# Kudo510/ImageSequenceRegistrationfor6DPoseEstimationLabeling

Hardware: AMD Instinct MI355X
Metric: registered images/sec (T-LESS obj 1-like, synthetic) + final Chamfer error (higher is better)
Workload: dtype bf16

## Files before the change

imagesequenceregistrationfor6dposeestimationlabeling_amd/csrc/nn_batched.hip:

```cpp
#include "isr_common.hpp"

#include <cstddef>
#include <cstdlib>

namespace {

#ifndef ISR_NN_PACKED_BATCH
#define ISR_NN_PACKED_BATCH 1
#endif
constexpr int kThreads = 256;
constexpr int kTile = 256;
constexpr int kGroup = 8;
constexpr int kNV = 18;

__device__ __forceinline__ void xform64(const double* __restrict__ T, float x, float y, float z,
                                        double& ox, double& oy, double& oz) {
  if (T == nullptr) {
    ox = x; oy = y; oz = z;
    return;
  }
  const double dx = x, dy = y, dz = z;
  ox = fma(T[2], dz, fma(T[1], dy, fma(T[0], dx, T[3])));
  oy = fma(T[6], dz, fma(T[5], dy, fma(T[4], dx, T[7])));
  oz = fma(T[10], dz, fma(T[9], dy, fma(T[8], dx, T[11])));
}

constexpr int kUnresolved = -2;

template <int RQ>
__device__ __forceinline__ int query_of(int r) {
  return (int)blockIdx.x * RQ * kThreads + ((int)threadIdx.x >> 6) * (RQ * 64) + r * 64 + ((int)threadIdx.x & 63);
}

__global__ __launch_bounds__(256) void tile_box_kernel(const float* __restrict__ tgt, int Nt, float* __restrict__ box) {
  __shared__ float red[6][4];
  const int j = blockIdx.x * 256 + threadIdx.x;
  float v[6] = {3.0e38f, 3.0e38f, 3.0e38f, -3.0e38f, -3.0e38f, -3.0e38f};
  if (j < Nt) {
#pragma unroll
    for (int a = 0; a < 3; ++a) v[a] = v[3 + a] = tgt[3 * (size_t)j + a];
  }
#pragma unroll
  for (int a = 0; a < 3; ++a) {
#pragma unroll
    for (int o = 32; o >= 1; o >>= 1) {
      v[a] = fminf(v[a], __shfl_xor(v[a], o, 64));
      v[3 + a] = fmaxf(v[3 + a], __shfl_xor(v[3 + a], o, 64));
    }
  }
  if ((threadIdx.x & 63) == 0) {
#pragma unroll
    for (int a = 0; a < 6; ++a) red[a][threadIdx.x >> 6] = v[a];
  }
  __syncthreads();
  if (threadIdx.x < 6) {
    const int a = threadIdx.x;
    const float r0 = red[a][0], r1 = red[a][1], r2 = red[a][2], r3 = red[a][3];
    box[6 * (size_t)blockIdx.x + a] = a < 3 ? fminf(fminf(r0, r1), fminf(r2, r3)) : fmaxf(fmaxf(r0, r1), fmaxf(r2, r3));
  }
}

constexpr int kIcpItemDoubles = 20;
constexpr int kIcpStateInts = 8;
template <int RQ, bool FILTER, bool EXACT = false, bool CULL = false, bool ITEMS = false>
__global__ __launch_bounds__(kThreads) void nn_search_kernel(
    const float* __restrict__ qry, int Nq, const float* __restrict__ tgt, int Nt,
    const double* __restrict__ Tq, const double* __restrict__ Tt, int split_len, int nsplit,
    float* __restrict__ part_d2, int32_t* __restrict__ part_idx, const int32_t* __restrict__ skip,
    const int32_t* __restrict__ unresolved, unsigned long long* __restrict__ packed = nullptr,
    const int32_t* __restrict__ warm = nullptr, int32_t* __restrict__ amb = nullptr,
    const float* __restrict__ t2_bound = nullptr, const float* __restrict__ tile_box = nullptr, float cull_r2 = 0.f,
    size_t qry_item_stride = 0) {
  __shared__ __attribute__((aligned(16))) float lds[2][FILTER ? 4 : 3][kTile];
  __shared__ float tile_t2[2][kThreads / 64];
  if (ITEMS) {
    if (skip[(size_t)blockIdx.z * kIcpStateInts]) return;
    qry += (size_t)blockIdx.z * qry_item_stride;
  } else if (skip && *skip) {
    return;
  }
  if (unresolved && *unresolved == 0) return;

  const int tid = threadIdx.x;
  const int b = blockIdx.z;
  const int split = blockIdx.y;
  if (unresolved) {
    int mine = 0;
#pragma unroll
    for (int r = 0; r < RQ; ++r) {
      const int qi = query_of<RQ>(r);
      if (qi < Nq) mine |= part_idx[((size_t)b * nsplit + split) * Nq + qi] == kUnresolved;
// ... 326 lines not shown
      counted = (radius < 0.0) || (s2 <= radius * radius);
      if (counted) {
        v[0] = d; v[1] = s2; v[2] = 1.0;
        if (WANT_COV) {
          const double q[3] = {q0, q1, q2}, t[3] = {t0, t1, t2};
#pragma unroll
          for (int r = 0; r < 3; ++r) {
            v[3 + r] = q[r];
            v[6 + r] = t[r];
#pragma unroll
            for (int c = 0; c < 3; ++c) v[9 + 3 * r + c] = q[r] * t[c];
          }
        }
      }
    }
    if (nn_idx) nn_idx[(size_t)b * Nq + qi] = counted ? bi : -1;
    if (nn_d) nn_d[(size_t)b * Nq + qi] = d;
  }

  constexpr int nv = WANT_COV ? kNV : 3;
  const int wave = tid >> 6, lane = tid & 63;
#pragma unroll
  for (int k = 0; k < nv; ++k) {
    const double s = wave_sum(v[k]);
    if (lane == 0) red[wave][k] = s;
  }
  __syncthreads();
  if (tid < kNV) {
    double s = 0.0;
    if (tid < nv) s = ((red[0][tid] + red[1][tid]) + red[2][tid]) + red[3][tid];
    part_sums[((size_t)b * gridDim.x + blockIdx.x) * kNV + tid] = s;
  }
}

__global__ void nn_reduce_kernel(const double* __restrict__ part_sums, int nblk, int B,
                                 double* __restrict__ sum_d, double* __restrict__ sum_d2,
                                 int32_t* __restrict__ n_in, double* __restrict__ cov) {
  const int b = blockIdx.x * blockDim.y + threadIdx.y;
  const int k = threadIdx.x;
  if (b >= B || k >= kNV) return;
  double s = 0.0;
  for (int i = 0; i < nblk; ++i) s += part_sums[((size_t)b * nblk + i) * kNV + k];
  if (k == 0 && sum_d) sum_d[b] = s;
  if (k == 1 && sum_d2) sum_d2[b] = s;
  if (k == 2 && n_in) n_in[b] = (int32_t)s;
  if (k >= 3 && cov) cov[(size_t)b * 16 + (k - 3)] = s;
  if (k == 2 && cov) cov[(size_t)b * 16 + 15] = s;
}


__global__ __launch_bounds__(kThreads) void add_metric_kernel(const float* __restrict__ verts, int V,
                                                              const double* __restrict__ Ta,
                                                              const double* __restrict__ Tb,
                                                              double* __restrict__ out) {
  __shared__ double red[kThreads / 64];
  const int b = blockIdx.x;
  const double* ta = Ta ? Ta + 12 * (size_t)b : nullptr;
  const double* tb = Tb ? Tb + 12 * (size_t)b : nullptr;
  double s = 0.0;
  for (int i = threadIdx.x; i < V; i += kThreads) {
    const float x = verts[3 * (size_t)i], y = verts[3 * (size_t)i + 1], z = verts[3 * (size_t)i + 2];
    double a0, a1, a2, b0, b1, b2;
    xform64(ta, x, y, z, a0, a1, a2);
    xform64(tb, x, y, z, b0, b1, b2);
    const double ex = a0 - b0, ey = a1 - b1, ez = a2 - b2;
    s += sqrt(fma(ez, ez, fma(ey, ey, ex * ex)));
  }
  s = wave_sum(s);
  if ((threadIdx.x & 63) == 0) red[threadIdx.x >> 6] = s;
  __syncthreads();
  if (threadIdx.x == 0) out[b] = (((red[0] + red[1]) + red[2]) + red[3]) / (double)V;
}


struct IcpState {
  double prev_fit, prev_rmse;
  int32_t iter, done;
  int32_t ticket, pad;
};
static_assert(sizeof(IcpState) == kIcpStateInts * sizeof(int32_t) && offsetof(IcpState, done) == 5 * sizeof(int32_t),
              "nn_search_kernel<.., ITEMS> steps from one item's done flag to the next by kIcpStateInts");

__device__ void jacobi4_largest(double A[4][4], double q[4]) {
  double V[4][4] = {{1, 0, 0, 0}, {0, 1, 0, 0}, {0, 0, 1, 0}, {0, 0, 0, 1}};
  for (int sweep = 0; sweep < 16; ++sweep) {
    double off = 0.0, dia = 0.0;
#pragma unroll
    for (int p = 0; p < 4; ++p) {
      dia += A[p][p] * A[p][p];
#pragma unroll
      for (int r = p + 1; r < 4; ++r) off += A[p][r] * A[p][r];
    }
    if (off <= 1e-34 * dia) break;
#pragma unroll
    for (int p = 0; p < 3; ++p)
#pragma unroll
      for (int r = p + 1; r < 4; ++r) {
        if (A[p][r] != 0.0) {
          const double theta = (A[r][r] - A[p][p]) / (2.0 * A[p][r]);
          const double t = (theta >= 0 ? 1.0 : -1.0) / (fabs(theta) + sqrt(theta * theta + 1.0));
          const double c = 1.0 / sqrt(t * t + 1.0), sn = t * c;
#pragma unroll
          for (int k = 0; k < 4; ++k) {
            const double akp = A[k][p], akr = A[k][r];
            A[k][p] = c * akp - sn * akr;
            A[k][r] = sn * akp + c * akr;
          }
#pragma unroll
          for (int k = 0; k < 4; ++k) {
            const double apk = A[p][k], ark = A[r][k];
            A[p][k] = c * apk - sn * ark;
            A[r][k] = sn * apk + c * ark;
          }
#pragma unroll
          for (int k = 0; k < 4; ++k) {
            const double vkp = V[k][p], vkr = V[k][r];
            V[k][p] = c * vkp - sn * vkr;
            V[k][r] = sn * vkp + c * vkr;
          }
        }
      }
  }
  double lam = A[0][0];
#pragma unroll
  for (int k = 0; k < 4; ++k) q[k] = V[k][0];
#pragma unroll
  for (int j = 1; j < 4; ++j) {
    if (A[j][j] > lam) {
      lam = A[j][j];
#pragma unroll
      for (int k = 0; k < 4; ++k) q[k] = V[k][j];
    }
  }
}

constexpr int kIcpLanes = 16;

__device__ void icp_reduce_and_update(const double* __restrict__ part_sums, int nblk, int Ns, int max_iter,
                                      double rel_fitness, double rel_rmse, double* __restrict__ T,
                                      IcpState* __restrict__ st, double* __restrict__ result) {
  __shared__ double part[kNV][kIcpLanes];
  __shared__ double v[kNV];
  for (int idx = threadIdx.x; idx < kNV * kIcpLanes; idx += blockDim.x) {
    const int k = idx / kIcpLanes, l = idx % kIcpLanes;
    double s = 0.0;
    for (int i = l; i < nblk; i += kIcpLanes) s += part_sums[(size_t)i * kNV + k];
    part[k][l] = s;
  }
  __syncthreads();
  if (threadIdx.x < kNV) {
    double s = 0.0;
    for (int l = 0; l < kIcpLanes; ++l) s += part[threadIdx.x][l];
    v[threadIdx.x] = s;
  }
  __syncthreads();
  if (threadIdx.x != 0) return;
  const double n = v[2];
  const double fit = n / (double)Ns;
  const double rmse = n > 0 ? sqrt(v[1] / n) : 0.0;
  const int it = st->iter;
  result[0] = fit; result[1] = rmse; result[2] = (double)it; result[3] = n;
  const bool conv = it > 0 && fabs(st->prev_fit - fit) < rel_fitness && fabs(st->prev_rmse - rmse) < rel_rmse;
  if (conv || it >= max_iter || n < 3) { st->done = 1; return; }
  st->prev_fit = fit; st->prev_rmse = rmse; st->iter = it + 1;
  double mq[3], mt[3], S[3][3];
  for (int a = 0; a < 3; ++a) { mq[a] = v[3 + a] / n; mt[a] = v[6 + a] / n; }
  for (int a = 0; a < 3; ++a)
    for (int b = 0; b < 3; ++b) S[a][b] = v[9 + 3 * a + b] - n * mq[a] * mt[b];
  double N4[4][4] = {
      {S[0][0] + S[1][1] + S[2][2], S[1][2] - S[2][1], S[2][0] - S[0][2], S[0][1] - S[1][0]},
      {S[1][2] - S[2][1], S[0][0] - S[1][1] - S[2][2], S[0][1] + S[1][0], S[2][0] + S[0][2]},
      {S[2][0] - S[0][2], S[0][1] + S[1][0], -S[0][0] + S[1][1] - S[2][2], S[1][2] + S[2][1]},
      {S[0][1] - S[1][0], S[2][0] + S[0][2], S[1][2] + S[2][1], -S[0][0] - S[1][1] + S[2][2]}};
  double q[4];
  jacobi4_largest(N4, q);
  const double nq = 1.0 / sqrt(q[0] * q[0] + q[1] * q[1] + q[2] * q[2] + q[3] * q[3]);
  const double w = q[0] * nq, x = q[1] * nq, y = q[2] * nq, z = q[3] * nq;
  const double R[3][3] = {{1 - 2 * (y * y + z * z), 2 * (x * y - z * w), 2 * (x * z + y * w)},
                          {2 * (x * y + z * w), 1 - 2 * (x * x + z * z), 2 * (y * z - x * w)},
                          {2 * (x * z - y * w), 2 * (y * z + x * w), 1 - 2 * (x * x + y * y)}};
  double U[3][4];
  for (int a = 0; a < 3; ++a) {
    for (int b = 0; b < 3; ++b) U[a][b] = R[a][b];
    U[a][3] = mt[a] - (R[a][0] * mq[0] + R[a][1] * mq[1] + R[a][2] * mq[2]);
  }
  double Tn[12];
  for (int a = 0; a < 3; ++a)
    for (int b = 0; b < 4; ++b)
      Tn[4 * a + b] = U[a][0] * T[b] + U[a][1] * T[4 + b] + U[a][2] * T[8 + b] + (b == 3 ? U[a][3] : 0.0);
  for (int k = 0; k < 12; ++k) T[k] = Tn[k];
}

__global__ __launch_bounds__(kThreads) void icp_finalize_update_kernel(
    const float* __restrict__ src, int Ns, const float* __restrict__ tgt, int Nt, double radius,
    unsigned long long* __restrict__ packed, int32_t* __restrict__ prev_idx, int32_t* __restrict__ amb,
    double* __restrict__ part_sums, int max_iter,
    double rel_fitness, double rel_rmse, double* __restrict__ T, IcpState* __restrict__ st, double* __restrict__ result,
    size_t src_item_stride = 0, size_t out_item_stride = 0) {
  __shared__ double red[kThreads / 64][kNV];
  __shared__ int last;
  __shared__ int nflag, flist[kThreads];
  __shared__ double wd[4][kThreads / 64];
  __shared__ int wi[4][kThreads / 64];
  {
    const size_t b = blockIdx.y;
    src += b * src_item_stride;
    packed += b * Ns; prev_idx += b * Ns; amb += b * Ns;
    part_sums += b * gridDim.x * kNV;
    st += b;
    T += b * out_item_stride; result += b * out_item_stride;
  }
  if (st->done) return;
  const int tid = threadIdx.x;
  const int qi = blockIdx.x * kThreads + tid;
  if (tid == 0) nflag = 0;
  __syncthreads();
  if (qi < Ns && amb[qi]) {
    amb[qi] = 0;
    flist[atomicAdd(&nflag, 1)] = qi;
  }
  __syncthreads();
  const int nf = nflag;
  constexpr int kRes = 4;
  for (int f0 = 0; f0 < nf; f0 += kRes) {
    double qx[kRes], qy[kRes], qz[kRes], bd[kRes];
    int bi[kRes];
#pragma unroll
    for (int k = 0; k < kRes; ++k) {
      const int pq = flist[min(f0 + k, nf - 1)];
      xform64(T, src[3 * (size_t)pq], src[3 * (size_t)pq + 1], src[3 * (size_t)pq + 2], qx[k], qy[k], qz[k]);
      bd[k] = __builtin_inf();
      bi[k] = 0x7fffffff;
    }
#pragma unroll 4
    for (int j = tid; j < Nt; j += kThreads) {
      const double tx = tgt[3 * (size_t)j], ty = tgt[3 * (size_t)j + 1], tz = tgt[3 * (size_t)j + 2];
#pragma unroll
      for (int k = 0; k < kRes; ++k) {
        const double ex = qx[k] - tx, ey = qy[k] - ty, ez = qz[k] - tz;
        const double s2 = fma(ez, ez, fma(ey, ey, ex * ex));
        if (s2 < bd[k]) { bd[k] = s2; bi[k] = j; }
      }
    }
#pragma unroll
    for (int k = 0; k < kRes; ++k) {
#pragma unroll
      for (int off = 32; off > 0; off >>= 1) {
        const double od = __shfl_xor(bd[k], off, 64);
        const int oi = __shfl_xor(bi[k], off, 64);
        if (od < bd[k] || (od == bd[k] && oi < bi[k])) { bd[k] = od; bi[k] = oi; }
      }
      if ((tid & 63) == 0) { wd[k][tid >> 6] = bd[k]; wi[k][tid >> 6] = bi[k]; }
    }
    __syncthreads();
    if (tid < kRes && f0 + tid < nf) {
      double d = wd[tid][0];
      int i = wi[tid][0];
      for (int w = 1; w < kThreads / 64; ++w)
        if (wd[tid][w] < d || (wd[tid][w] == d && wi[tid][w] < i)) { d = wd[tid][w]; i = wi[tid][w]; }
      packed[flist[f0 + tid]] = ((unsigned long long)__float_as_uint((float)d) << 32) | (unsigned int)i;
    }
    __syncthreads();
  }
  double v[kNV];
#pragma unroll
  for (int k = 0; k < kNV; ++k) v[k] = 0.0;
  if (qi < Ns) {
    const unsigned long long pk = packed[qi];
    packed[qi] = ~0ull;
    prev_idx[qi] = pk != ~0ull ? (int)(unsigned int)pk : -1;
    if (pk != ~0ull) {
      const int bi = (int)(unsigned int)pk;
      double q0, q1, q2;
      xform64(T, src[3 * (size_t)qi], src[3 * (size_t)qi + 1], src[3 * (size_t)qi + 2], q0, q1, q2);
      const double t0 = tgt[3 * (size_t)bi], t1 = tgt[3 * (size_t)bi + 1], t2 = tgt[3 * (size_t)bi + 2];
      const double ex = q0 - t0, ey = q1 - t1, ez = q2 - t2;
      const double s2 = fma(ez, ez, fma(ey, ey, ex * ex));
      if (s2 <= radius * radius) {
        v[0] = sqrt(s2); v[1] = s2; v[2] = 1.0;
        const double q[3] = {q0, q1, q2}, t[3] = {t0, t1, t2};
#pragma unroll
        for (int r = 0; r < 3; ++r) {
          v[3 + r] = q[r];
          v[6 + r] = t[r];
#pragma unroll
          for (int c = 0; c < 3; ++c) v[9 + 3 * r + c] = q[r] * t[c];
        }
      }
    }
  }
  const int wave = tid >> 6, lane = tid & 63;
#pragma unroll
  for (int k = 0; k < kNV; ++k) {
    const double s = wave_sum(v[k]);
    if (lane == 0) red[wave][k] = s;
  }
  __syncthreads();
  if (tid < kNV) part_sums[(size_t)blockIdx.x * kNV + tid] = ((red[0][tid] + red[1][tid]) + red[2][tid]) + red[3][tid];
  __threadfence();
  __syncthreads();
  if (tid == 0) last = (atomicAdd(&st->ticket, 1) == (int)gridDim.x - 1);
  __syncthreads();
  if (!last) return;
  __threadfence();
  if (tid == 0) st->ticket = 0;
  icp_reduce_and_update(part_sums, gridDim.x, Ns, max_iter, rel_fitness, rel_rmse, T, st, result);
}

__global__ void icp_init_kernel(IcpState* st, double* T, unsigned long long* packed, int32_t* amb, int Ns,
                                size_t out_item_stride = 0) {
  const size_t b = blockIdx.y;
  const int i = blockIdx.x * blockDim.x + threadIdx.x;
  if (i < Ns) { packed[b * Ns + i] = ~0ull; amb[b * Ns + i] = 0; }
  if (i != 0) return;
  st += b; T += b * out_item_stride;
  st->prev_fit = 0; st->prev_rmse = 0; st->iter = 0; st->done = 0; st->ticket = 0;
  T[12] = 0; T[13] = 0; T[14] = 0; T[15] = 1;
}

__global__ __launch_bounds__(kThreads) void cloud_r2max_kernel(const float* __restrict__ tgt, int Nt, float* __restrict__ out) {
  __shared__ float red[kThreads / 64];
  float m = 0.f;
  for (int j = threadIdx.x; j < Nt; j += kThreads) {
    const float x = tgt[3 * (size_t)j], y = tgt[3 * (size_t)j + 1], z = tgt[3 * (size_t)j + 2];
    m = fmaxf(m, __builtin_fmaf(z, z, __builtin_fmaf(y, y, x * x)));
  }
#pragma unroll
  for (int o = 32; o >= 1; o >>= 1) m = fmaxf(m, __shfl_xor(m, o, 64));
  if ((threadIdx.x & 63) == 0) red[threadIdx.x >> 6] = m;
  __syncthreads();
  if (threadIdx.x == 0) *out = 1.0001f * fmaxf(fmaxf(red[0], red[1]), fmaxf(red[2], red[3]));
}

struct NNPlan {
  int rq;
  int qblocks;
  int nsplit;
  int split_len;
  int fblocks;
  int bchunk;
  bool grid;
  bool tile;
};

constexpr size_t kPartBudget = size_t(192) << 20;

NNPlan make_plan(int Nq, int Nt, int B, bool brute_only = false) {
  NNPlan p;
  p.rq = (Nq >= 4 * kThreads) ? 4 : 1;
  const int rq_knob = isr::tuning(ISR_TUNE_NN_PLAN_RQ);
  const long want_env = isr::tuning(ISR_TUNE_NN_PLAN_BLOCKS);
  if (rq_knob == 1 || rq_knob == 4) p.rq = rq_knob;
  p.qblocks = (Nq + p.rq * kThreads - 1) / (p.rq * kThreads);
#ifndef ISR_NN_WANT_BLOCKS
#define ISR_NN_WANT_BLOCKS 4096
#endif
  const long want = want_env > 0 ? want_env : ISR_NN_WANT_BLOCKS;
  long ns = (want + (long)p.qblocks * B - 1) / ((long)p.qblocks * B);
  const int max_split = (Nt + kTile - 1) / kTile;
  if (ns < 1) ns = 1;
  if (ns > max_split) ns = max_split;
  int tiles_per_split = (max_split + (int)ns - 1) / (int)ns;
  p.split_len = tiles_per_split * kTile;
  p.nsplit = (Nt + p.split_len - 1) / p.split_len;
  p.fblocks = (Nq + kThreads - 1) / kThreads;
  p.grid = false;
  p.tile = B >= 4 && Nq >= 1024 && Nt >= 4096 && (long)Nq * B >= (1L << 17);
  if (const int path = isr::tuning(ISR_TUNE_NN_PATH); path >= 0) { p.grid = path == 1; p.tile = path == 2; }
  if (brute_only) p.grid = p.tile = false;
  if (p.grid || p.tile) {
    p.nsplit = 1;
    p.split_len = max_split * kTile;
  }
  const size_t per_b = (size_t)p.nsplit * Nq * 8;
  long bc = (long)(kPartBudget / (per_b ? per_b : 1));
  if (bc < 1) bc = 1;
  if (bc > B) bc = B;
  if (bc > 65535) bc = 65535;
  p.bchunk = (int)bc;
  return p;
}

constexpr int kFilterMinTiles = 4;
void launch_search(const NNPlan& p, const dim3& grid, hipStream_t stream, const float* qry, int Nq, const float* tgt, int Nt,
                   const double* tq, const double* tt, float* part_d2, int32_t* part_idx, const int32_t* skip,
                   const int32_t* unresolved, unsigned long long* packed, const int32_t* warm, int32_t* amb = nullptr,
                   const float* t2_bound = nullptr, const float* tile_box = nullptr, float cull_r2 = 0.f,
                   bool items = false, size_t qry_item_stride = 0) {
  bool filter = warm != nullptr || p.split_len >= kFilterMinTiles * kTile;
  if (const int f = isr::tuning(ISR_TUNE_NN_FILTER); f >= 0 && !warm) filter = f == 1;
#define ISR_SEARCH(RQv, Fv)                                                                                              \
  nn_search_kernel<RQv, Fv><<<grid, kThreads, 0, stream>>>(qry, Nq, tgt, Nt, tq, tt, p.split_len, p.nsplit, part_d2, part_idx, \
                                                           skip, unresolved, packed, warm)
#define ISR_SEARCH_X(RQv, Fv)                                                                                            \
  nn_search_kernel<RQv, Fv, true, Fv><<<grid, kThreads, 0, stream>>>(qry, Nq, tgt, Nt, tq, tt, p.split_len, p.nsplit, part_d2, \
                                                                     part_idx, skip, unresolved, packed, warm, amb, t2_bound, tile_box, cull_r2)
#define ISR_SEARCH_ITEMS(RQv, Fv)                                                                                        \
  nn_search_kernel<RQv, Fv, true, Fv, true><<<grid, kThreads, 0, stream>>>(qry, Nq, tgt, Nt, tq, tt, p.split_len, p.nsplit,    \
                                                                           part_d2, part_idx, skip, unresolved, packed, warm, \
                                                                           amb, t2_bound, tile_box, cull_r2, qry_item_stride)
  if (items) {
    if (p.rq == 4) { if (filter) ISR_SEARCH_ITEMS(4, true); else ISR_SEARCH_ITEMS(4, false); }
    else { if (filter) ISR_SEARCH_ITEMS(1, true); else ISR_SEARCH_ITEMS(1, false); }
    return;
  }
  if (amb) {
    if (p.rq == 4) { if (filter) ISR_SEARCH_X(4, true); else ISR_SEARCH_X(4, false); }
    else { if (filter) ISR_SEARCH_X(1, true); else ISR_SEARCH_X(1, false); }
    return;
  }
  if (p.rq == 4) { if (filter) ISR_SEARCH(4, true); else ISR_SEARCH(4, false); }
  else { if (filter) ISR_SEARCH(1, true); else ISR_SEARCH(1, false); }
#undef ISR_SEARCH_ITEMS
#undef ISR_SEARCH_X
#undef ISR_SEARCH
}

}

extern "C" size_t isr_nn_batched_workspace_bytes(int Nq, int Nt, int B) {
  if (Nq <= 0 || Nt <= 0 || B <= 0) return 0;
  const NNPlan p = make_plan(Nq, Nt, B);
  size_t n = 0;
  n += isr::align_up((size_t)p.bchunk * p.nsplit * Nq * sizeof(float), 256);
  n += isr::align_up((size_t)p.bchunk * p.nsplit * Nq * sizeof(int32_t), 256);
  n += isr::align_up((size_t)B * p.fblocks * kNV * sizeof(double), 256);
  if (p.grid) n += grid_ws_bytes(Nt);
  if (p.tile) n += tile_ws_bytes(Nq, Nt);
  return n + 256;
}

extern "C" int isr_nn_batched(const float* qry, int Nq, const float* tgt, int Nt, const double* Tq,
// ... 19 lines not shown
  TileWs tw{};
  if (p.grid) {
    gw = take_grid(w, Nt);
    build_grid(gw, tgt, Nt, stream);
    ISR_CHECK_LAUNCH("grid build");
  }
  if (p.tile) {
    tw = take_tile(w, Nq, Nt);
    build_tile(tw, qry, Nq, tgt, Nt, stream);
    ISR_CHECK_LAUNCH("tile grid build");
  }
  const float stop_radius = (radius >= 0.0 && !nn_d) ? (float)(radius * (1.0 + 1e-6)) : -1.f;

  for (int b0 = 0; b0 < B; b0 += p.bchunk) {
    const int nb = (B - b0 < p.bchunk) ? (B - b0) : p.bchunk;
    const double* tq = Tq ? Tq + 12 * (size_t)b0 : nullptr;
    const double* tt = Tt ? Tt + 12 * (size_t)b0 : nullptr;
    const dim3 grid(p.qblocks, p.nsplit, nb);
    const int32_t* unres = nullptr;
    if (p.grid) {
      nn_grid_search_kernel<<<dim3(p.fblocks, nb), kThreads, 0, stream>>>(qry, Nq, gw.desc, gw.start, gw.sorted, tq, tt,
                                                                          stop_radius, part_d2, part_idx,
                                                                          gw.unresolved, nullptr);
      ISR_CHECK_LAUNCH("nn_grid_search_kernel");
      unres = gw.unresolved;
    }
    unsigned long long* packed = nullptr;
    if (!p.tile && !p.grid && p.nsplit > 1 && ISR_NN_PACKED_BATCH) {
      packed = reinterpret_cast<unsigned long long*>(part_d2);
      ISR_CHECK_HIP(hipMemsetAsync(packed, 0xFF, (size_t)nb * Nq * sizeof(unsigned long long), stream));
    }
    if (p.tile)
      launch_tile_search(tw, Nq, Nt, tq, tt, nb, stop_radius, part_d2, part_idx, nullptr, stream);
    else
      launch_search(p, grid, stream, qry, Nq, tgt, Nt, tq, tt, packed ? nullptr : part_d2, packed ? nullptr : part_idx, nullptr, unres,
                    packed, nullptr);
    ISR_CHECK_LAUNCH("nn_search_kernel");
    const dim3 fgrid(p.fblocks, nb);
    if (cov)
      nn_finalize_kernel<true><<<fgrid, kThreads, 0, stream>>>(qry, Nq, tgt, Tq, Tt, p.nsplit,
                                                               radius, part_d2, part_idx, b0,
                                                               nn_idx, nn_d, part_sums, nullptr, packed);
    else
      nn_finalize_kernel<false><<<fgrid, kThreads, 0, stream>>>(qry, Nq, tgt, Tq, Tt, p.nsplit,
                                                                radius, part_d2, part_idx, b0,
                                                                nn_idx, nn_d, part_sums, nullptr, packed);
    ISR_CHECK_LAUNCH("nn_finalize_kernel");
  }
  if (sum_d || sum_d2 || n_in || cov) {
    const dim3 rblock(32, 8);
    nn_reduce_kernel<<<(B + 7) / 8, rblock, 0, stream>>>(part_sums, p.fblocks, B, sum_d, sum_d2,
                                                         n_in, cov);
    ISR_CHECK_LAUNCH("nn_reduce_kernel");
  }
  return ISR_OK;
}

extern "C" int isr_add_metric(const float* verts, int V, const double* Ta, const double* Tb, int B,
                              double* mean_out, isr_stream_t stream) {
  ISR_REQUIRE(verts && mean_out, "isr_add_metric: null pointer");
  ISR_REQUIRE(V > 0 && B > 0, "isr_add_metric: V=%d B=%d", V, B);
  add_metric_kernel<<<B, kThreads, 0, isr::as_stream(stream)>>>(verts, V, Ta, Tb, mean_out);
  ISR_CHECK_LAUNCH("add_metric_kernel");
  return ISR_OK;
}

extern "C" size_t isr_icp_workspace_bytes(int Ns, int Nt) {
  if (Ns <= 0 || Nt <= 0) return 0;
  const NNPlan p = make_plan(Ns, Nt, 1, true);
  return isr::align_up((size_t)p.fblocks * kNV * sizeof(double), 256) + isr::align_up((size_t)Ns * 8, 256) +
         2 * isr::align_up((size_t)Ns * 4, 256) + isr::align_up((size_t)((Nt + kTile - 1) / kTile) * 6 * sizeof(float), 256) + 2048;
}

extern "C" int isr_icp_point_to_point(const float* src, int Ns, const float* tgt, int Nt, double threshold,
                                      int max_iter, double rel_fitness, double rel_rmse, double* T_io,
                                      double* result, void* ws, size_t ws_bytes, isr_stream_t stream_) {
  ISR_REQUIRE(src && tgt && T_io && result, "isr_icp_point_to_point: null pointer");
  ISR_REQUIRE(Ns > 0 && Nt > 0 && max_iter >= 0 && threshold > 0, "isr_icp_point_to_point: Ns=%d Nt=%d max_iter=%d", Ns, Nt, max_iter);
  if (!ws || ws_bytes < isr_icp_workspace_bytes(Ns, Nt)) {
    isr::set_error("isr_icp_point_to_point: workspace %zu < %zu", ws_bytes, isr_icp_workspace_bytes(Ns, Nt));
    return ISR_ERR_WORKSPACE;
  }
  hipStream_t stream = isr::as_stream(stream_);
  const NNPlan p = make_plan(Ns, Nt, 1, true);
  isr::Workspace w(ws, ws_bytes);
  double* part_sums = w.take<double>((size_t)p.fblocks * kNV);
  IcpState* st = w.take<IcpState>(1);
  unsigned long long* packed = w.take<unsigned long long>(Ns);
  int32_t* prev_idx = w.take<int32_t>(Ns);
  int32_t* amb = w.take<int32_t>(Ns);
  float* t2_bound = w.take<float>(1);
  float* tile_box = w.take<float>((size_t)((Nt + kTile - 1) / kTile) * 6);
  const bool warm = isr::tuning(ISR_TUNE_ICP_WARM) != 0;
  icp_init_kernel<<<(Ns + kThreads - 1) / kThreads, kThreads, 0, stream>>>(st, T_io, packed, amb, Ns);
  cloud_r2max_kernel<<<1, kThreads, 0, stream>>>(tgt, Nt, t2_bound);
#ifndef ISR_ICP_CULL
#define ISR_ICP_CULL 1
#endif
  const float cull_r2 = (float)(threshold * threshold * 1.0001 + 1e-6);
  if (ISR_ICP_CULL) tile_box_kernel<<<(Nt + kTile - 1) / kTile, 256, 0, stream>>>(tgt, Nt, tile_box);
  const dim3 grid(p.qblocks, p.nsplit, 1);
  for (int it = 0; it <= max_iter; ++it) {
    const int32_t* w_idx = (it > 0 && warm) ? prev_idx : nullptr;
    launch_search(p, grid, stream, src, Ns, tgt, Nt, T_io, nullptr, nullptr, nullptr, &st->done, nullptr, packed, w_idx, amb,
                  t2_bound, ISR_ICP_CULL ? tile_box : nullptr, cull_r2);
    icp_finalize_update_kernel<<<p.fblocks, kThreads, 0, stream>>>(src, Ns, tgt, Nt, threshold, packed, prev_idx, amb, part_sums,
                                                                   max_iter, rel_fitness, rel_rmse, T_io, st, result);
  }
  ISR_CHECK_LAUNCH("icp kernels");
  return ISR_OK;
}

extern "C" size_t isr_icp_point_to_point_batch_workspace_bytes(int Ns, int Nt, int B) {
  if (Ns <= 0 || Nt <= 0 || B <= 0) return 0;
  const NNPlan p = make_plan(Ns, Nt, B, true);
  return isr::align_up((size_t)B * p.fblocks * kNV * sizeof(double), 256) + isr::align_up((size_t)B * sizeof(IcpState), 256) +
         isr::align_up((size_t)B * Ns * 8, 256) + 2 * isr::align_up((size_t)B * Ns * 4, 256) +
         isr::align_up((size_t)((Nt + kTile - 1) / kTile) * 6 * sizeof(float), 256) + 2048;
}

extern "C" int isr_icp_point_to_point_batch(const float* src, size_t src_item_stride, int Ns, const float* tgt, int Nt, int B,
                                            double threshold, int max_iter, double rel_fitness, double rel_rmse,
                                            double* state, void* ws, size_t ws_bytes, isr_stream_t stream_) {
  ISR_REQUIRE(src && tgt && state, "isr_icp_point_to_point_batch: null pointer");
  ISR_REQUIRE(Ns > 0 && Nt > 0 && B >= 0 && B <= 65535, "isr_icp_point_to_point_batch: Ns=%d Nt=%d must be positive, B=%d in [0, 65535]",
              Ns, Nt, B);
  ISR_REQUIRE(threshold > 0 && max_iter >= 0, "isr_icp_point_to_point_batch: threshold=%g must be positive, max_iter=%d non-negative",
              threshold, max_iter);
  ISR_REQUIRE(src_item_stride == 0 || src_item_stride >= 3 * (size_t)Ns,
              "isr_icp_point_to_point_batch: src_item_stride=%zu must be 0 (one source for all items) or at least 3*Ns=%zu floats",
              src_item_stride, 3 * (size_t)Ns);
  if (B == 0) return ISR_OK;
  if (!ws || ws_bytes < isr_icp_point_to_point_batch_workspace_bytes(Ns, Nt, B)) {
    isr::set_error("isr_icp_point_to_point_batch: workspace %zu < %zu", ws_bytes,
                   isr_icp_point_to_point_batch_workspace_bytes(Ns, Nt, B));
    return ISR_ERR_WORKSPACE;
  }
  hipStream_t stream = isr::as_stream(stream_);
  const NNPlan p = make_plan(Ns, Nt, B, true);
  isr::Workspace w(ws, ws_bytes);
  double* part_sums = w.take<double>((size_t)B * p.fblocks * kNV);
  IcpState* st = w.take<IcpState>(B);
  unsigned long long* packed = w.take<unsigned long long>((size_t)B * Ns);
  int32_t* prev_idx = w.take<int32_t>((size_t)B * Ns);
  int32_t* amb = w.take<int32_t>((size_t)B * Ns);
  float* t2_bound = w.take<float>(1);
  float* tile_box = w.take<float>((size_t)((Nt + kTile - 1) / kTile) * 6);
  const bool warm = isr::tuning(ISR_TUNE_ICP_WARM) != 0;
  icp_init_kernel<<<dim3((Ns + kThreads - 1) / kThreads, B), kThreads, 0, stream>>>(st, state, packed, amb, Ns, kIcpItemDoubles);
  cloud_r2max_kernel<<<1, kThreads, 0, stream>>>(tgt, Nt, t2_bound);
  const float cull_r2 = (float)(threshold * threshold * 1.0001 + 1e-6);
  if (ISR_ICP_CULL) tile_box_kernel<<<(Nt + kTile - 1) / kTile, 256, 0, stream>>>(tgt, Nt, tile_box);
  const dim3 grid(p.qblocks, p.nsplit, B);
  for (int it = 0; it <= max_iter; ++it) {
    const int32_t* w_idx = (it > 0 && warm) ? prev_idx : nullptr;
    launch_search(p, grid, stream, src, Ns, tgt, Nt, state, nullptr, nullptr, nullptr, &st->done, nullptr, packed, w_idx, amb,
                  t2_bound, ISR_ICP_CULL ? tile_box : nullptr, cull_r2, true, src_item_stride);
    icp_finalize_update_kernel<<<dim3(p.fblocks, B), kThreads, 0, stream>>>(src, Ns, tgt, Nt, threshold, packed, prev_idx, amb,
                                                                             part_sums, max_iter, rel_fitness, rel_rmse, state,
                                                                             st, state + 16, src_item_stride, kIcpItemDoubles);
  }
  ISR_CHECK_LAUNCH("icp batch kernels");
  return ISR_OK;
}
```

imagesequenceregistrationfor6dposeestimationlabeling_amd/csrc/ransac.hip:

```cpp
#include "isr_common.hpp"
#include "p3p_device.hpp"
#include "ransac_seq.hpp"

namespace {

using namespace isr_p3p;

constexpr int kMaxBatch = 16;
constexpr int kChainMax = 128;

struct ImgBatch {
  Cam cam[kMaxBatch];
  uint32_t seed_lo[kMaxBatch], seed_hi[kMaxBatch];
};

struct ImgDev {
  Cam cam;
  uint32_t seed_lo, seed_hi;
};

__global__ void set_imgs_kernel(ImgBatch ib, int nb, ImgDev* __restrict__ dst) {
  const int b = threadIdx.x;
  if (b >= nb) return;
  dst[b].cam = ib.cam[b];
  dst[b].seed_lo = ib.seed_lo[b];
  dst[b].seed_hi = ib.seed_hi[b];
}

__device__ __forceinline__ void p3p_body(const float* __restrict__ p3d, const float* __restrict__ p2d,
                                         const int32_t* __restrict__ M_dev, int M_cap, const ImgDev& img, int H,
                                         double* __restrict__ Rt_out, uint8_t* __restrict__ ok_out,
                                         int32_t* __restrict__ sample_out) {
  const int b = blockIdx.z;
  const Cam& cam = img.cam;
  const uint32_t seed_lo = img.seed_lo, seed_hi = img.seed_hi;
  p3d += (size_t)b * M_cap * 3; p2d += (size_t)b * M_cap * 2;
  Rt_out += (size_t)b * H * 12; ok_out += (size_t)b * H;
  if (sample_out) sample_out += (size_t)b * H * 4;
  const int h = blockIdx.x * blockDim.x + threadIdx.x;
  if (h >= H) return;
  const int M = M_dev[b];
  double* Rt = Rt_out + 12 * (size_t)h;
  uint8_t ok = 0;
  int s[4] = {0, 0, 0, 0};
  if (M >= 4) {
    uint32_t rnd[4];
    philox4x32_10((uint32_t)h, 0u, 0u, 0u, seed_lo, seed_hi, rnd);
#pragma unroll
    for (int j = 0; j < 4; ++j) s[j] = (int)(((uint64_t)rnd[j] * (uint64_t)M) >> 32);
    const bool distinct = s[0] != s[1] && s[0] != s[2] && s[0] != s[3] && s[1] != s[2] && s[1] != s[3] && s[2] != s[3];
    P3PIn in;
#pragma unroll
    for (int j = 0; j < 3; ++j) {
      in.x[j] = {(double)p3d[3 * (size_t)s[j]], (double)p3d[3 * (size_t)s[j] + 1], (double)p3d[3 * (size_t)s[j] + 2]};
      const double u = p2d[2 * (size_t)s[j]], v = p2d[2 * (size_t)s[j] + 1];
      V3 y = {cam.ki[0] * u + cam.ki[1] * v + cam.ki[2], cam.ki[3] * u + cam.ki[4] * v + cam.ki[5],
              cam.ki[6] * u + cam.ki[7] * v + cam.ki[8]};
      in.y[j] = scale(y, 1.0 / sqrt(dot(y, y)));
    }
    double lam[4][3];
    const int n = distinct ? p3p_depths(in, lam) : 0;
    const V3 X4 = {(double)p3d[3 * (size_t)s[3]], (double)p3d[3 * (size_t)s[3] + 1], (double)p3d[3 * (size_t)s[3] + 2]};
    const double u4 = p2d[2 * (size_t)s[3]], v4 = p2d[2 * (size_t)s[3] + 1];
    double best = 1e300;
    for (int i = 0; i < n; ++i) {
      double cand[12];
      if (!pose_from_depths(in, lam[i], cand)) continue;
      const double xc = cand[0] * X4.x + cand[1] * X4.y + cand[2] * X4.z + cand[3];
      const double yc = cand[4] * X4.x + cand[5] * X4.y + cand[6] * X4.z + cand[7];
      const double zc = cand[8] * X4.x + cand[9] * X4.y + cand[10] * X4.z + cand[11];
      if (!(zc > 0.0)) continue;
      const double px = cam.k[0] * xc + cam.k[1] * yc + cam.k[2] * zc;
      const double py = cam.k[3] * xc + cam.k[4] * yc + cam.k[5] * zc;
      const double pz = cam.k[6] * xc + cam.k[7] * yc + cam.k[8] * zc;
      const double eu = px / pz - u4, ev = py / pz - v4;
      const double e = eu * eu + ev * ev;
      if (e < best) {
        best = e;
        ok = 1;
#pragma unroll
        for (int k = 0; k < 12; ++k) Rt[k] = cand[k];
      }
    }
// ... 313 lines not shown
    mask[w] = (lane == 0) ? (uint32_t)bal : (uint32_t)(bal >> 32);
}

#ifndef ISR_GN_SPLIT_SOLVE
#define ISR_GN_SPLIT_SOLVE 1
#endif
constexpr int kRefThreads = 256;
#ifndef ISR_GN_STOP_ROT2
#define ISR_GN_STOP_ROT2 1e-18
#endif
#ifndef ISR_GN_STOP_TRANS2
#define ISR_GN_STOP_TRANS2 1e-14
#endif
constexpr double kGnStopRot2 = ISR_GN_STOP_ROT2, kGnStopTrans2 = ISR_GN_STOP_TRANS2;
#ifndef ISR_REF_BLOCKS
#define ISR_REF_BLOCKS 64
#endif
constexpr int kRefBlocks = ISR_REF_BLOCKS;
constexpr int kNAcc = 29;

__device__ void gn_solve(const double* __restrict__ partial, int nblocks, double* __restrict__ Rt, int32_t* __restrict__ state) {
  __shared__ double s[kNAcc];
  if (threadIdx.x < kNAcc) {
    double a = 0.0;
    for (int b = 0; b < nblocks; ++b) a += partial[(size_t)b * kNAcc + threadIdx.x];
    s[threadIdx.x] = a;
  }
  __syncthreads();
  if (threadIdx.x != 0) return;
  if (s[28] < 4.0) { state[0] = 1; return; }
  double A[6][6], g[6];
  int k = 0;
  for (int i = 0; i < 6; ++i)
    for (int j = i; j < 6; ++j) { A[i][j] = s[k]; A[j][i] = s[k]; ++k; }
  for (int i = 0; i < 6; ++i) g[i] = -s[21 + i];
  double tr = 0.0;
  for (int i = 0; i < 6; ++i) tr += A[i][i];
  for (int i = 0; i < 6; ++i) A[i][i] += 1e-14 * tr;
  double L[6][6];
  for (int i = 0; i < 6; ++i)
    for (int j = 0; j < 6; ++j) L[i][j] = 0.0;
  for (int j = 0; j < 6; ++j) {
    double d = A[j][j];
    for (int p = 0; p < j; ++p) d -= L[j][p] * L[j][p];
    if (!(d > 0.0)) { state[0] = 1; return; }
    L[j][j] = sqrt(d);
    for (int i = j + 1; i < 6; ++i) {
      double v = A[i][j];
      for (int p = 0; p < j; ++p) v -= L[i][p] * L[j][p];
      L[i][j] = v / L[j][j];
    }
  }
  double y[6], x[6];
  for (int i = 0; i < 6; ++i) {
    double v = g[i];
    for (int p = 0; p < i; ++p) v -= L[i][p] * y[p];
    y[i] = v / L[i][i];
  }
  for (int i = 5; i >= 0; --i) {
    double v = y[i];
    for (int p = i + 1; p < 6; ++p) v -= L[p][i] * x[p];
    x[i] = v / L[i][i];
  }
  const double hx = 0.5 * x[0], hy = 0.5 * x[1], hz = 0.5 * x[2];
  const double nrm = 1.0 / sqrt(1.0 + hx * hx + hy * hy + hz * hz);
  const double qw = nrm, qx = hx * nrm, qy = hy * nrm, qz = hz * nrm;
  const double Q[9] = {1 - 2 * (qy * qy + qz * qz), 2 * (qx * qy - qz * qw), 2 * (qx * qz + qy * qw),
                       2 * (qx * qy + qz * qw), 1 - 2 * (qx * qx + qz * qz), 2 * (qy * qz - qx * qw),
                       2 * (qx * qz - qy * qw), 2 * (qy * qz + qx * qw), 1 - 2 * (qx * qx + qy * qy)};
  double T[12], O[12];
  for (int i = 0; i < 12; ++i) T[i] = Rt[i];
  for (int r = 0; r < 3; ++r) {
    for (int c = 0; c < 4; ++c) O[4 * r + c] = Q[3 * r] * T[c] + Q[3 * r + 1] * T[4 + c] + Q[3 * r + 2] * T[8 + c];
    O[4 * r + 3] += x[3 + r];
  }
  for (int i = 0; i < 12; ++i) Rt[i] = O[i];
  const double dw = x[0] * x[0] + x[1] * x[1] + x[2] * x[2];
  const double dt = x[3] * x[3] + x[4] * x[4] + x[5] * x[5];
  const double tt = O[3] * O[3] + O[7] * O[7] + O[11] * O[11];
  if (dw < kGnStopRot2 && dt < kGnStopTrans2 * (tt + 1.0)) state[0] = 1;
}


__device__ __forceinline__ void gn_point(const double (&T)[12], const Cam& cam, double X, double Y, double Z, double ox, double oy,
                                         double (&acc)[kNAcc]) {
  const double xc = __builtin_fma(T[0], X, __builtin_fma(T[1], Y, __builtin_fma(T[2], Z, T[3])));
  const double yc = __builtin_fma(T[4], X, __builtin_fma(T[5], Y, __builtin_fma(T[6], Z, T[7])));
  const double zc = __builtin_fma(T[8], X, __builtin_fma(T[9], Y, __builtin_fma(T[10], Z, T[11])));
  const double px = __builtin_fma(cam.k[0], xc, __builtin_fma(cam.k[1], yc, cam.k[2] * zc));
  const double py = __builtin_fma(cam.k[3], xc, __builtin_fma(cam.k[4], yc, cam.k[5] * zc));
  const double pz = __builtin_fma(cam.k[6], xc, __builtin_fma(cam.k[7], yc, cam.k[8] * zc));
  const double ipz = 1.0 / pz;
  const double u = px * ipz, v = py * ipz;
  const double ru = u - ox, rv = v - oy;
  const double a0 = __builtin_fma(-u, cam.k[6], cam.k[0]) * ipz, a1 = __builtin_fma(-u, cam.k[7], cam.k[1]) * ipz,
               a2 = __builtin_fma(-u, cam.k[8], cam.k[2]) * ipz;
  const double b0 = __builtin_fma(-v, cam.k[6], cam.k[3]) * ipz, b1 = __builtin_fma(-v, cam.k[7], cam.k[4]) * ipz,
               b2 = __builtin_fma(-v, cam.k[8], cam.k[5]) * ipz;
  const double Ju[6] = {__builtin_fma(a2, yc, -(a1 * zc)), __builtin_fma(a0, zc, -(a2 * xc)), __builtin_fma(a1, xc, -(a0 * yc)), a0, a1, a2};
  const double Jv[6] = {__builtin_fma(b2, yc, -(b1 * zc)), __builtin_fma(b0, zc, -(b2 * xc)), __builtin_fma(b1, xc, -(b0 * yc)), b0, b1, b2};
  int k = 0;
#pragma unroll
  for (int i = 0; i < 6; ++i)
#pragma unroll
    for (int j = i; j < 6; ++j) { acc[k] = __builtin_fma(Ju[i], Ju[j], __builtin_fma(Jv[i], Jv[j], acc[k])); ++k; }
#pragma unroll
  for (int i = 0; i < 6; ++i) acc[21 + i] = __builtin_fma(Ju[i], ru, __builtin_fma(Jv[i], rv, acc[21 + i]));
  acc[27] = __builtin_fma(ru, ru, __builtin_fma(rv, rv, acc[27]));
  acc[28] += 1.0;
}

__global__ __launch_bounds__(kRefThreads) void gn_accumulate_kernel(
    const float* __restrict__ p3d, const float* __restrict__ p2d, const int32_t* __restrict__ M_dev, int M_cap,
    const uint32_t* __restrict__ mask, int mask_words, const ImgDev* __restrict__ ib, const double* __restrict__ Rt,
    const int32_t* __restrict__ status_dev, int32_t* __restrict__ state,
    double* __restrict__ partial) {
  __shared__ double red[kRefThreads / 64][kNAcc];
  __shared__ int last;
  const int img = blockIdx.z;
  const Cam& cam = ib[img].cam;
  p3d += (size_t)img * M_cap * 3; p2d += (size_t)img * M_cap * 2;
  if (mask) mask += (size_t)img * mask_words;
  Rt += (size_t)img * 12; state += 4 * img; partial += (size_t)img * kRefBlocks * kNAcc;
  if (state[0]) return;
  if (status_dev && status_dev[img] == 0) return;
  double acc[kNAcc];
#pragma unroll
  for (int i = 0; i < kNAcc; ++i) acc[i] = 0.0;
  const int M = M_dev[img];
  const bool live = (status_dev == nullptr) || (status_dev[img] != 0);
  if (live) {
    double T[12];
#pragma unroll
    for (int i = 0; i < 12; ++i) T[i] = Rt[i];
    for (int m = blockIdx.x * kRefThreads + threadIdx.x; m < M; m += kRefBlocks * kRefThreads) {
      if (mask && !((mask[m >> 5] >> (m & 31)) & 1u)) continue;
      gn_point(T, cam, p3d[3 * (size_t)m], p3d[3 * (size_t)m + 1], p3d[3 * (size_t)m + 2], p2d[2 * (size_t)m], p2d[2 * (size_t)m + 1], acc);
    }
  }
  const int wave = threadIdx.x >> 6, lane = threadIdx.x & 63;
#pragma unroll
  for (int i = 0; i < kNAcc; ++i) {
    double s = acc[i];
#pragma unroll
    for (int off = 32; off > 0; off >>= 1) s += __shfl_down(s, off, 64);
    if (lane == 0) red[wave][i] = s;
  }
  __syncthreads();
  if (threadIdx.x < kNAcc)
    partial[(size_t)blockIdx.x * kNAcc + threadIdx.x] =
        ((red[0][threadIdx.x] + red[1][threadIdx.x]) + red[2][threadIdx.x]) + red[3][threadIdx.x];
#if ISR_GN_SPLIT_SOLVE
  (void)last;
}

__global__ __launch_bounds__(64) void gn_solve_kernel(const double* __restrict__ partial, int nblocks, double* __restrict__ Rt,
                                                       const int32_t* __restrict__ status_dev, int32_t* __restrict__ state) {
  const int img = blockIdx.x;
  state += 4 * img;
  if (state[0]) return;
  if (status_dev && status_dev[img] == 0) return;
  gn_solve(partial + (size_t)img * kRefBlocks * kNAcc, nblocks, Rt + (size_t)img * 12, state);
}
#else
  __threadfence();
  __syncthreads();
  if (threadIdx.x == 0) last = (atomicAdd(&state[1], 1) == (int)gridDim.x - 1);
  __syncthreads();
  if (!last) return;
  __threadfence();
  if (threadIdx.x == 0) state[1] = 0;
  gn_solve(partial, (int)gridDim.x, const_cast<double*>(Rt), state);
}
#endif

constexpr int kSmallM = 8192;

__global__ __launch_bounds__(kRefThreads) void gn_small_kernel(
    const float* __restrict__ p3d, const float* __restrict__ p2d, const int32_t* __restrict__ M_dev, int M_cap,
    uint32_t* __restrict__ mask, int mask_words, const ImgDev* __restrict__ ib, int iters, float reperr,
    double* __restrict__ pose, const int32_t* __restrict__ status_dev) {
  __shared__ double red[kRefThreads / 64][kNAcc];
  __shared__ double part[kNAcc];
  __shared__ double Ts[12];
  __shared__ float Pm[12];
  __shared__ int32_t st[2];
  const int img = blockIdx.x, tid = threadIdx.x;
  if (status_dev && status_dev[img] == 0) return;
  const Cam& cam = ib[img].cam;
  p3d += (size_t)img * M_cap * 3; p2d += (size_t)img * M_cap * 2;
  mask += (size_t)img * mask_words; pose += (size_t)img * 12;
  const int M = M_dev[img];
  if (tid < 12) Ts[tid] = pose[tid];
  __syncthreads();
  auto remask = [&]() {
    if (tid < 12) {
      const int r = tid / 4, c = tid % 4;
      Pm[tid] = (float)fma(cam.k[3 * r + 2], Ts[8 + c], fma(cam.k[3 * r + 1], Ts[4 + c], cam.k[3 * r] * Ts[c]));
    }
    __syncthreads();
    for (int m0 = 0; m0 < M_cap; m0 += kRefThreads) {
      const int m = m0 + tid;
      bool in = false;
      if (m < M)
        in = inlier_f32(Pm, p3d[3 * (size_t)m], p3d[3 * (size_t)m + 1], p3d[3 * (size_t)m + 2], p2d[2 * (size_t)m],
                        p2d[2 * (size_t)m + 1], reperr);
      const unsigned long long bal = __ballot(in);
      const int lane = tid & 63, w = m >> 5;
      if ((lane == 0 || lane == 32) && w < (M_cap + 31) / 32) mask[w] = (lane == 0) ? (uint32_t)bal : (uint32_t)(bal >> 32);
    }
    __syncthreads();
  };
  for (int round = 0; round < 2; ++round) {
    if (round == 1) remask();
    if (tid == 0) { st[0] = 0; st[1] = 0; }
    __syncthreads();
    for (int it = 0; it < iters; ++it) {
      if (st[0]) break;
      double acc[kNAcc];
#pragma unroll
      for (int i = 0; i < kNAcc; ++i) acc[i] = 0.0;
      double T[12];
#pragma unroll
      for (int i = 0; i < 12; ++i) T[i] = Ts[i];
      for (int m = tid; m < M; m += kRefThreads) {
        if (!((mask[m >> 5] >> (m & 31)) & 1u)) continue;
        gn_point(T, cam, p3d[3 * (size_t)m], p3d[3 * (size_t)m + 1], p3d[3 * (size_t)m + 2], p2d[2 * (size_t)m], p2d[2 * (size_t)m + 1], acc);
      }
      const int wave = tid >> 6, lane = tid & 63;
#pragma unroll
// ... 400 lines not shown
```

Measured before the change: 1101.

## Reduce register pressure in ICP update, NN search and Gauss-Newton accumulation

```diff
diff --git a/imagesequenceregistrationfor6dposeestimationlabeling_amd/csrc/nn_batched.hip b/imagesequenceregistrationfor6dposeestimationlabeling_amd/csrc/nn_batched.hip
--- a/imagesequenceregistrationfor6dposeestimationlabeling_amd/csrc/nn_batched.hip
+++ b/imagesequenceregistrationfor6dposeestimationlabeling_amd/csrc/nn_batched.hip
@@ -7,6 +7,15 @@
 
 #ifndef ISR_NN_PACKED_BATCH
 #define ISR_NN_PACKED_BATCH 1
+#endif
+#ifndef ISR_ICP_UPDATE_SLICE
+#define ISR_ICP_UPDATE_SLICE 1
+#endif
+#ifndef ISR_NN_WARM_SLICE
+#define ISR_NN_WARM_SLICE 1
+#endif
+#ifndef ISR_NN_COLD_SLICE
+#define ISR_NN_COLD_SLICE 1
 #endif
 constexpr int kThreads = 256;
 constexpr int kTile = 256;
@@ -499,7 +508,15 @@
               "nn_search_kernel<.., ITEMS> steps from one item's done flag to the next by kIcpStateInts");
 
 __device__ void jacobi4_largest(double A[4][4], double q[4]) {
+#if ISR_ICP_UPDATE_SLICE
+  __shared__ double V[4][4];
+#pragma unroll
+  for (int p = 0; p < 4; ++p)
+#pragma unroll
+    for (int r = 0; r < 4; ++r) V[p][r] = p == r ? 1.0 : 0.0;
+#else
   double V[4][4] = {{1, 0, 0, 0}, {0, 1, 0, 0}, {0, 0, 1, 0}, {0, 0, 0, 1}};
+#endif
   for (int sweep = 0; sweep < 16; ++sweep) {
     double off = 0.0, dia = 0.0;
 #pragma unroll
@@ -591,6 +608,10 @@
       {S[0][1] - S[1][0], S[2][0] + S[0][2], S[1][2] + S[2][1], -S[0][0] - S[1][1] + S[2][2]}};
   double q[4];
   jacobi4_largest(N4, q);
+#if ISR_ICP_UPDATE_SLICE
+  __asm__ volatile("" ::: "memory");
+  for (int a = 0; a < 3; ++a) { mq[a] = v[3 + a] / v[2]; mt[a] = v[6 + a] / v[2]; }
+#endif
   const double nq = 1.0 / sqrt(q[0] * q[0] + q[1] * q[1] + q[2] * q[2] + q[3] * q[3]);
   const double w = q[0] * nq, x = q[1] * nq, y = q[2] * nq, z = q[3] * nq;
   const double R[3][3] = {{1 - 2 * (y * y + z * z), 2 * (x * y - z * w), 2 * (x * z + y * w)},
@@ -608,7 +629,12 @@
   for (int k = 0; k < 12; ++k) T[k] = Tn[k];
 }
 
-__global__ __launch_bounds__(kThreads) void icp_finalize_update_kernel(
+#if ISR_ICP_UPDATE_SLICE
+#define ISR_ICP_UPDATE_ATTR __attribute__((amdgpu_waves_per_eu(6)))
+#else
+#define ISR_ICP_UPDATE_ATTR
+#endif
+__global__ __launch_bounds__(kThreads) ISR_ICP_UPDATE_ATTR void icp_finalize_update_kernel(
     const float* __restrict__ src, int Ns, const float* __restrict__ tgt, int Nt, double radius,
     unsigned long long* __restrict__ packed, int32_t* __restrict__ prev_idx, int32_t* __restrict__ amb,
     double* __restrict__ part_sums, int max_iter,
@@ -649,7 +675,11 @@
       bd[k] = __builtin_inf();
       bi[k] = 0x7fffffff;
     }
+#if ISR_ICP_UPDATE_SLICE
+#pragma unroll 2
+#else
 #pragma unroll 4
+#endif
     for (int j = tid; j < Nt; j += kThreads) {
       const double tx = tgt[3 * (size_t)j], ty = tgt[3 * (size_t)j + 1], tz = tgt[3 * (size_t)j + 2];
 #pragma unroll
@@ -679,6 +709,38 @@
     }
     __syncthreads();
   }
+#if ISR_ICP_UPDATE_SLICE
+  double pq[3] = {0.0, 0.0, 0.0}, pt[3] = {0.0, 0.0, 0.0}, ps2 = 0.0;
+  bool counted = false;
+  if (qi < Ns) {
+    const unsigned long long pk = packed[qi];
+    packed[qi] = ~0ull;
+    prev_idx[qi] = pk != ~0ull ? (int)(unsigned int)pk : -1;
+    if (pk != ~0ull) {
+      const int bi = (int)(unsigned int)pk;
+      xform64(T, src[3 * (size_t)qi], src[3 * (size_t)qi + 1], src[3 * (size_t)qi + 2], pq[0], pq[1], pq[2]);
+      pt[0] = tgt[3 * (size_t)bi]; pt[1] = tgt[3 * (size_t)bi + 1]; pt[2] = tgt[3 * (size_t)bi + 2];
+      const double ex = pq[0] - pt[0], ey = pq[1] - pt[1], ez = pq[2] - pt[2];
+      ps2 = fma(ez, ez, fma(ey, ey, ex * ex));
+      counted = ps2 <= radius * radius;
+    }
+  }
+  const int wave = tid >> 6, lane = tid & 63;
+#pragma unroll
+  for (int k = 0; k < kNV; ++k) {
+    double vk;
+    if (k == 0) vk = sqrt(ps2);
+    else if (k == 1) vk = ps2;
+    else if (k == 2) vk = 1.0;
+    else if (k < 6) vk = pq[k - 3];
+    else if (k < 9) vk = pt[k - 6];
+    else vk = pq[(k - 9) / 3] * pt[(k - 9) % 3];
+    const double s = wave_sum(counted ? vk : 0.0);
+    if (lane == 0) red[wave][k] = s;
+  }
+  __syncthreads();
+  if (tid < kNV) part_sums[(size_t)blockIdx.x * kNV + tid] = ((red[0][tid] + red[1][tid]) + red[2][tid]) + red[3][tid];
+#else
   double v[kNV];
 #pragma unroll
   for (int k = 0; k < kNV; ++k) v[k] = 0.0;
@@ -714,6 +776,7 @@
   }
   __syncthreads();
   if (tid < kNV) part_sums[(size_t)blockIdx.x * kNV + tid] = ((red[0][tid] + red[1][tid]) + red[2][tid]) + red[3][tid];
+#endif
   __threadfence();
   __syncthreads();
   if (tid == 0) last = (atomicAdd(&st->ticket, 1) == (int)gridDim.x - 1);
@@ -762,9 +825,10 @@
 
 constexpr size_t kPartBudget = size_t(192) << 20;
 
-NNPlan make_plan(int Nq, int Nt, int B, bool brute_only = false) {
+NNPlan make_plan(int Nq, int Nt, int B, bool brute_only = false, int slice_rq = 0) {
   NNPlan p;
   p.rq = (Nq >= 4 * kThreads) ? 4 : 1;
+  if (p.rq == 4 && slice_rq > 0) p.rq = slice_rq;
   const int rq_knob = isr::tuning(ISR_TUNE_NN_PLAN_RQ);
   const long want_env = isr::tuning(ISR_TUNE_NN_PLAN_BLOCKS);
   if (rq_knob == 1 || rq_knob == 4) p.rq = rq_knob;
@@ -950,7 +1014,8 @@
     return ISR_ERR_WORKSPACE;
   }
   hipStream_t stream = isr::as_stream(stream_);
-  const NNPlan p = make_plan(Ns, Nt, 1, true);
+  const NNPlan p = make_plan(Ns, Nt, 1, true, ISR_NN_WARM_SLICE ? 1 : 0);
+  const NNPlan p_cold = make_plan(Ns, Nt, 1, true, ISR_NN_COLD_SLICE ? 1 : 0);
   isr::Workspace w(ws, ws_bytes);
   double* part_sums = w.take<double>((size_t)p.fblocks * kNV);
   IcpState* st = w.take<IcpState>(1);
@@ -967,11 +1032,11 @@
 #endif
   const float cull_r2 = (float)(threshold * threshold * 1.0001 + 1e-6);
   if (ISR_ICP_CULL) tile_box_kernel<<<(Nt + kTile - 1) / kTile, 256, 0, stream>>>(tgt, Nt, tile_box);
-  const dim3 grid(p.qblocks, p.nsplit, 1);
+  const dim3 grid(p.qblocks, p.nsplit, 1), grid_cold(p_cold.qblocks, p_cold.nsplit, 1);
   for (int it = 0; it <= max_iter; ++it) {
     const int32_t* w_idx = (it > 0 && warm) ? prev_idx : nullptr;
-    launch_search(p, grid, stream, src, Ns, tgt, Nt, T_io, nullptr, nullptr, nullptr, &st->done, nullptr, packed, w_idx, amb,
-                  t2_bound, ISR_ICP_CULL ? tile_box : nullptr, cull_r2);
+    launch_search(w_idx ? p : p_cold, w_idx ? grid : grid_cold, stream, src, Ns, tgt, Nt, T_io, nullptr, nullptr, nullptr,
+                  &st->done, nullptr, packed, w_idx, amb, t2_bound, ISR_ICP_CULL ? tile_box : nullptr, cull_r2);
     icp_finalize_update_kernel<<<p.fblocks, kThreads, 0, stream>>>(src, Ns, tgt, Nt, threshold, packed, prev_idx, amb, part_sums,
                                                                    max_iter, rel_fitness, rel_rmse, T_io, st, result);
   }
@@ -1005,7 +1070,8 @@
     return ISR_ERR_WORKSPACE;
   }
   hipStream_t stream = isr::as_stream(stream_);
-  const NNPlan p = make_plan(Ns, Nt, B, true);
+  const NNPlan p = make_plan(Ns, Nt, B, true, ISR_NN_WARM_SLICE ? 1 : 0);
+  const NNPlan p_cold = make_plan(Ns, Nt, B, true, ISR_NN_COLD_SLICE ? 1 : 0);
   isr::Workspace w(ws, ws_bytes);
   double* part_sums = w.take<double>((size_t)B * p.fblocks * kNV);
   IcpState* st = w.take<IcpState>(B);
@@ -1019,11 +1085,12 @@
   cloud_r2max_kernel<<<1, kThreads, 0, stream>>>(tgt, Nt, t2_bound);
   const float cull_r2 = (float)(threshold * threshold * 1.0001 + 1e-6);
   if (ISR_ICP_CULL) tile_box_kernel<<<(Nt + kTile - 1) / kTile, 256, 0, stream>>>(tgt, Nt, tile_box);
-  const dim3 grid(p.qblocks, p.nsplit, B);
+  const dim3 grid(p.qblocks, p.nsplit, B), grid_cold(p_cold.qblocks, p_cold.nsplit, B);
   for (int it = 0; it <= max_iter; ++it) {
     const int32_t* w_idx = (it > 0 && warm) ? prev_idx : nullptr;
-    launch_search(p, grid, stream, src, Ns, tgt, Nt, state, nullptr, nullptr, nullptr, &st->done, nullptr, packed, w_idx, amb,
-                  t2_bound, ISR_ICP_CULL ? tile_box : nullptr, cull_r2, true, src_item_stride);
+    launch_search(w_idx ? p : p_cold, w_idx ? grid : grid_cold, stream, src, Ns, tgt, Nt, state, nullptr, nullptr, nullptr,
+                  &st->done, nullptr, packed, w_idx, amb, t2_bound, ISR_ICP_CULL ? tile_box : nullptr, cull_r2, true,
+                  src_item_stride);
     icp_finalize_update_kernel<<<dim3(p.fblocks, B), kThreads, 0, stream>>>(src, Ns, tgt, Nt, threshold, packed, prev_idx, amb,
                                                                              part_sums, max_iter, rel_fitness, rel_rmse, state,
                                                                              st, state + 16, src_item_stride, kIcpItemDoubles);
diff --git a/imagesequenceregistrationfor6dposeestimationlabeling_amd/csrc/ransac.hip b/imagesequenceregistrationfor6dposeestimationlabeling_amd/csrc/ransac.hip
--- a/imagesequenceregistrationfor6dposeestimationlabeling_amd/csrc/ransac.hip
+++ b/imagesequenceregistrationfor6dposeestimationlabeling_amd/csrc/ransac.hip
@@ -1,4 +1,6 @@
 #include "isr_common.hpp"
+
+#include <type_traits>
 #include "p3p_device.hpp"
 #include "ransac_seq.hpp"
 
@@ -478,8 +480,9 @@
 }
 
 
+template <int K0 = 0, int K1 = 29>
 __device__ __forceinline__ void gn_point(const double (&T)[12], const Cam& cam, double X, double Y, double Z, double ox, double oy,
-                                         double (&acc)[kNAcc]) {
+                                         double (&acc)[29]) {
   const double xc = __builtin_fma(T[0], X, __builtin_fma(T[1], Y, __builtin_fma(T[2], Z, T[3])));
   const double yc = __builtin_fma(T[4], X, __builtin_fma(T[5], Y, __builtin_fma(T[6], Z, T[7])));
   const double zc = __builtin_fma(T[8], X, __builtin_fma(T[9], Y, __builtin_fma(T[10], Z, T[11])));
@@ -499,14 +502,27 @@
 #pragma unroll
   for (int i = 0; i < 6; ++i)
 #pragma unroll
-    for (int j = i; j < 6; ++j) { acc[k] = __builtin_fma(Ju[i], Ju[j], __builtin_fma(Jv[i], Jv[j], acc[k])); ++k; }
-#pragma unroll
-  for (int i = 0; i < 6; ++i) acc[21 + i] = __builtin_fma(Ju[i], ru, __builtin_fma(Jv[i], rv, acc[21 + i]));
-  acc[27] = __builtin_fma(ru, ru, __builtin_fma(rv, rv, acc[27]));
-  acc[28] += 1.0;
-}
-
-__global__ __launch_bounds__(kRefThreads) void gn_accumulate_kernel(
+    for (int j = i; j < 6; ++j) {
+      if (k >= K0 && k < K1) acc[k] = __builtin_fma(Ju[i], Ju[j], __builtin_fma(Jv[i], Jv[j], acc[k]));
+      ++k;
+    }
+#pragma unroll
+  for (int i = 0; i < 6; ++i)
+    if (21 + i >= K0 && 21 + i < K1) acc[21 + i] = __builtin_fma(Ju[i], ru, __builtin_fma(Jv[i], rv, acc[21 + i]));
+  if (27 >= K0 && 27 < K1) acc[27] = __builtin_fma(ru, ru, __builtin_fma(rv, rv, acc[27]));
+  if (28 >= K0 && 28 < K1) acc[28] += 1.0;
+}
+
+#ifndef ISR_GN_ACC_SLICE
+#define ISR_GN_ACC_SLICE 1
+#endif
+constexpr int kNAccHalf = 14;
+#if ISR_GN_ACC_SLICE
+#define ISR_GN_ACC_ATTR __attribute__((amdgpu_waves_per_eu(6)))
+#else
+#define ISR_GN_ACC_ATTR
+#endif
+__global__ __launch_bounds__(kRefThreads) ISR_GN_ACC_ATTR void gn_accumulate_kernel(
     const float* __restrict__ p3d, const float* __restrict__ p2d, const int32_t* __restrict__ M_dev, int M_cap,
     const uint32_t* __restrict__ mask, int mask_words, const ImgDev* __restrict__ ib, const double* __restrict__ Rt,
     const int32_t* __restrict__ status_dev, int32_t* __restrict__ state,
@@ -520,6 +536,36 @@
   Rt += (size_t)img * 12; state += 4 * img; partial += (size_t)img * kRefBlocks * kNAcc;
   if (state[0]) return;
   if (status_dev && status_dev[img] == 0) return;
+#if ISR_GN_ACC_SLICE
+  const int M = M_dev[img];
+  const bool live = (status_dev == nullptr) || (status_dev[img] != 0);
+  const int wave = threadIdx.x >> 6, lane = threadIdx.x & 63;
+  auto walk = [&](auto half) {
+    constexpr int K0 = decltype(half)::value ? kNAccHalf : 0, K1 = decltype(half)::value ? kNAcc : kNAccHalf;
+    double acc[kNAcc];
+#pragma unroll
+    for (int i = 0; i < kNAcc; ++i) acc[i] = 0.0;
+    if (live) {
+      double T[12];
+#pragma unroll
+      for (int i = 0; i < 12; ++i) T[i] = Rt[i];
+      for (int m = blockIdx.x * kRefThreads + threadIdx.x; m < M; m += kRefBlocks * kRefThreads) {
+        if (mask && !((mask[m >> 5] >> (m & 31)) & 1u)) continue;
+        gn_point<K0, K1>(T, cam, p3d[3 * (size_t)m], p3d[3 * (size_t)m + 1], p3d[3 * (size_t)m + 2], p2d[2 * (size_t)m],
+                         p2d[2 * (size_t)m + 1], acc);
+      }
+    }
+#pragma unroll
+    for (int i = K0; i < K1; ++i) {
+      double s = acc[i];
+#pragma unroll
+      for (int off = 32; off > 0; off >>= 1) s += __shfl_down(s, off, 64);
+      if (lane == 0) red[wave][i] = s;
+    }
+  };
+  walk(std::integral_constant<int, 0>{});
+  walk(std::integral_constant<int, 1>{});
+#else
   double acc[kNAcc];
 #pragma unroll
   for (int i = 0; i < kNAcc; ++i) acc[i] = 0.0;
@@ -542,6 +588,7 @@
     for (int off = 32; off > 0; off >>= 1) s += __shfl_down(s, off, 64);
     if (lane == 0) red[wave][i] = s;
   }
+#endif
   __syncthreads();
   if (threadIdx.x < kNAcc)
     partial[(size_t)blockIdx.x * kNAcc + threadIdx.x] =
```

After: 1104, median of 6. Within noise of the previous version (+0.3%).
